# Audio-WestlakeU/FullSubNet

Measured on AMD Instinct MI355X. Metric: frames/sec (16 kHz, 512-FFT, hop 256), whole job, higher is better.
Workload: dtype f32

## Files before the change

fullsubnet_amd/csrc/fb_chain_kernels.hip:

```cpp
#include "fsn_common.h"

namespace {

constexpr int CHMAX = 512;
constexpr int CFS = CHMAX / 4;
constexpr int CREP = 16;

struct ChainArgs {
    const float* gx0;
    const float* whh0_p;
    const float* wih1_p;
    const float* whh1_p;
    const float* b1;
    float* hx0;
    float* hx1;
    float* gx1;
    float* hseq1;
    float* hseq0;
    float* gates0;
    float* cseq0;
    float* gates1;
    float* cseq1;
    unsigned* flags;
    unsigned* status;
    unsigned long long spin_ticks;
    int Tp, RT, Npad;
};

__device__ __forceinline__ bool chain_wait(const unsigned* flags, int nflags, unsigned epoch, const unsigned* one,
                                           unsigned one_epoch, unsigned* status, unsigned long long ticks) {
    const int lane = threadIdx.x & 63;
    const unsigned long long* f = reinterpret_cast<const unsigned long long*>(flags) + lane;
    unsigned long long t0 = 0;
    for (unsigned spins = 0;; ++spins) {
        unsigned long long v = ~0ull;
        unsigned w = ~0u;
        if (epoch > 0 && 2 * lane < nflags) v = __hip_atomic_load(f, __ATOMIC_RELAXED, __HIP_MEMORY_SCOPE_AGENT);
        if (one && lane == 0) w = __hip_atomic_load(one, __ATOMIC_RELAXED, __HIP_MEMORY_SCOPE_AGENT);
        if (__all((int)((unsigned)v >= epoch && (unsigned)(v >> 32) >= epoch && w >= one_epoch))) return true;
        if ((spins & 255u) == 255u && fsn_wait_give_up(status, spins, t0, ticks, 1u + epoch)) return false;
    }
}

typedef unsigned u32x4 __attribute__((ext_vector_type(4)));
__device__ __forceinline__ void chain_store16(const __amdgpu_buffer_rsrc_t& r, unsigned voff, unsigned soff, f32x4 v) {
    __builtin_amdgcn_raw_buffer_store_b128(__builtin_bit_cast(u32x4, v), r, voff, soff, 16);
}
template <int Q>
__device__ __forceinline__ float quad_bcast(float v) {
    return __builtin_bit_cast(float, __builtin_amdgcn_mov_dpp(__builtin_bit_cast(int, v), Q * 0x55, 0xf, 0xf, true));
}

template <int CH, int KS, bool SAVE = false, int CELL = 0>
__global__ __launch_bounds__(256, 1) void fb_chain_kernel(const ChainArgs a) {
    static_assert(!(SAVE && CELL != 0), "the training form is built for the LSTM cell");
    constexpr int CKC = CH / 16;
    constexpr int CNW = CH / 4;
    static_assert(CKC % 4 == 0 && CNW % 2 == 0 && CNW <= CFS, "hidden size: a multiple of 64, at most 512");
    constexpr int RTW = 4 / KS;
    constexpr int CW = CKC / KS;
    __shared__ f32x4 red[KS > 1 ? (KS - 1) * RTW * 64 : 1];

    const int stage = (int)blockIdx.x / CNW, j = (int)blockIdx.x % CNW;
    const int lane = threadIdx.x & 63, wave = __builtin_amdgcn_readfirstlane(threadIdx.x >> 6);
    const int rt = wave % RTW, kp = wave / RTW;
    const int lr = lane & 15, lq = lane >> 4, g = lr >> 2, ul = lr & 3;
    const int Tp = a.Tp, RT = a.RT;
    const bool active = rt < RT, owner = active && kp == 0;

    unsigned* fl0 = a.flags;
    unsigned* fl1 = a.flags + CREP * CFS;
    const int rep = j % CREP;

    const __amdgpu_buffer_rsrc_t r0 = __builtin_amdgcn_make_buffer_rsrc(a.hx0, 0, 0x7fffffff, 0x00020000);
    const __amdgpu_buffer_rsrc_t r1 = __builtin_amdgcn_make_buffer_rsrc(a.hx1, 0, 0x7fffffff, 0x00020000);
    const __amdgpu_buffer_rsrc_t rx = __builtin_amdgcn_make_buffer_rsrc(a.gx1, 0, 0x7fffffff, 0x00020000);
    const unsigned lane16 = (unsigned)lane * 16u;

    auto load_w = [&](const float* packed, f32x4 (&w)[CW]) {
        const float* wp = packed + ((size_t)(g * CKC + (j >> 2)) * CKC * 64 + lq * 16 + 4 * (j & 3) + ul) * 4;
#pragma unroll
        for (int q = 0; q < CW; ++q) w[q] = *reinterpret_cast<const f32x4*>(wp + (size_t)(kp * CW + q) * 256);
    };
    auto load_a = [&](f32x4 (&ar)[CW], const __amdgpu_buffer_rsrc_t& r, int ts) {
        const unsigned base = (unsigned)((((size_t)ts * RT + rt) * CKC + kp * CW) * 1024);
#pragma unroll
        for (int q = 0; q < CW; ++q)
            ar[q] = __builtin_bit_cast(f32x4, __builtin_amdgcn_raw_buffer_load_b128(r, lane16, base + q * 1024u, 16));
        __builtin_amdgcn_sched_barrier(0);
    };
    auto mac = [&](f32x4 acc, const f32x4 (&ar)[CW], const f32x4 (&w)[CW]) -> f32x4 {
#pragma unroll
        for (int q = 0; q < CW; ++q)
#pragma unroll
            for (int jj = 0; jj < 4; ++jj) acc = mfma16(ar[q][jj], w[q][jj], acc);
        return acc;
    };
    auto reduce = [&](f32x4 acc) -> f32x4 {
        if (KS > 1) {
            if (kp > 0) red[((kp - 1) * RTW + rt) * 64 + lane] = acc;
            __syncthreads();
            if (kp == 0) {
#pragma unroll
                for (int p = 1; p < KS; ++p) {
                    const f32x4 o = red[((p - 1) * RTW + rt) * 64 + lane];
                    acc = f32x4{acc[0] + o[0], acc[1] + o[1], acc[2] + o[2], acc[3] + o[3]};
                }
            }
        }
        return acc;
    };
    auto publish = [&](unsigned* flags, unsigned epoch) {
        asm volatile("s_waitcnt vmcnt(0)" ::: "memory");
        __syncthreads();
        if ((int)threadIdx.x < CREP)
            __hip_atomic_store(flags + (size_t)threadIdx.x * CFS + j, epoch, __ATOMIC_RELAXED, __HIP_MEMORY_SCOPE_AGENT);
    };
    auto quad_transpose = [&](const float (&v)[4]) -> f32x4 {
        f32x4 o;
#pragma unroll
        for (int u = 0; u < 4; ++u) {
            const float t0 = u == 0 ? quad_bcast<0>(v[0]) : u == 1 ? quad_bcast<1>(v[0]) : u == 2 ? quad_bcast<2>(v[0]) : quad_bcast<3>(v[0]);
            const float t1 = u == 0 ? quad_bcast<0>(v[1]) : u == 1 ? quad_bcast<1>(v[1]) : u == 2 ? quad_bcast<2>(v[1]) : quad_bcast<3>(v[1]);
            const float t2 = u == 0 ? quad_bcast<0>(v[2]) : u == 1 ? quad_bcast<1>(v[2]) : u == 2 ? quad_bcast<2>(v[2]) : quad_bcast<3>(v[2]);
            const float t3 = u == 0 ? quad_bcast<0>(v[3]) : u == 1 ? quad_bcast<1>(v[3]) : u == 2 ? quad_bcast<2>(v[3]) : quad_bcast<3>(v[3]);
            o[u] = ul == 0 ? t0 : ul == 1 ? t1 : ul == 2 ? t2 : t3;
        }
        return o;
    };
    const int hrow = 4 * lq + ul;
    auto cell = [&](f32x4 acc, float (&c)[4], float* gates_t, float* cseq_t) -> f32x4 {
        float act[4], hq[4];
        if constexpr (CELL == 1) {
#pragma unroll
            for (int i = 0; i < 4; ++i) {
                const float v = g < 2 ? sigmoid_f(acc[i]) : acc[i];
                const float z = __shfl(v, lane + 4, 64);
                const float nx = __shfl(v, lane + 8, 64);
                const float nh = __shfl(v, lane + 12, 64);
                const float n = tanhf(nx + v * nh);
                const float hn = n + z * (c[i] - n);
                c[i] = hn;
                hq[i] = hn;
            }
            return quad_transpose(hq);
        }
#pragma unroll
        for (int i = 0; i < 4; ++i) act[i] = g == 2 ? tanh_fast(acc[i]) : sigmoid_fast(acc[i]);
#pragma unroll
        for (int i = 0; i < 4; ++i) {
            const float fg = __shfl(act[i], lane + 4, 64);
            const float gg = __shfl(act[i], lane + 8, 64);
            const float og = __shfl(act[i], lane + 12, 64);
            const float cn = fg * c[i] + act[i] * gg;
            c[i] = cn;
            hq[i] = og * tanh_fast(cn);
        }
        if (SAVE) {
            const size_t row = (size_t)rt * 16 + hrow;
            *reinterpret_cast<f32x4*>(gates_t + row * (4 * CH) + g * CH + 4 * j) = quad_transpose(act);
            const f32x4 cv = quad_transpose(c);
            if (g == 0) *reinterpret_cast<f32x4*>(cseq_t + row * CH + 4 * j) = cv;
        }
        return quad_transpose(hq);
    };
    const unsigned hvoff = (unsigned)(((j & 3) * 16 + hrow) * 16);
    auto hsoff = [&](int t) { return (unsigned)((((size_t)t * RT + rt) * CKC + (j >> 2)) * 1024); };
    const unsigned gx1_wave = (unsigned)(((size_t)j * 4 + wave) * 1024);
    const unsigned gx1_step = (unsigned)CNW * 4096u;
    float c[4] = {0.f, 0.f, 0.f, 0.f};

    if (stage == 0) {
        f32x4 whh[CW], wih[CW], ar[CW];
        load_w(a.whh0_p, whh);
        load_w(a.wih1_p, wih);
        const float bias1 = a.b1[g * CH + 4 * j + ul];
        const float* gx0p = a.gx0 + ((size_t)(g * CKC + (j >> 2)) * 64 + lq * 16 + 4 * (j & 3) + ul) * 4 +
                            (size_t)rt * (4 * CKC) * 256;
        const size_t gx0_step = (size_t)RT * (4 * CKC) * 256;
        f32x4 gxn = f32x4{0.f, 0.f, 0.f, 0.f};
        if (owner) gxn = *reinterpret_cast<const f32x4*>(gx0p);
        for (int t = 0; t <= Tp; ++t) {
            f32x4 acc = gxn;
            if (owner && t + 1 < Tp) gxn = *reinterpret_cast<const f32x4*>(gx0p + (size_t)(t + 1) * gx0_step);
            if (t > 0) {
                if (wave == 0) (void)chain_wait(fl0 + rep * CFS, CNW, (unsigned)t, nullptr, 0, a.status, a.spin_ticks);
                __syncthreads();
                if (active) load_a(ar, r0, t - 1);
            }
            if (t < Tp) {
                if (active && t > 0) acc = mac(acc, ar, whh);
                acc = reduce(acc);
                if (owner) {
                    const f32x4 hv = cell(acc, c, SAVE ? a.gates0 + (size_t)t * a.Npad * 4 * CH : nullptr,
                                          SAVE ? a.cseq0 + (size_t)t * a.Npad * CH : nullptr);
                    if (g == 0) {
                        chain_store16(r0, hvoff, hsoff(t), hv);
                        if (SAVE) *reinterpret_cast<f32x4*>(a.hseq0 + ((size_t)t * a.Npad + rt * 16 + hrow) * CH + 4 * j) = hv;
                    }
                }
            }
            const bool proj = t > 0 && active;
            const float b = kp == 0 ? bias1 : 0.f;
            if (t < Tp) publish(fl0, (unsigned)t + 1);
            if (proj) {
                const f32x4 accx = mac(f32x4{b, b, b, b}, ar, wih);
                const unsigned so = (unsigned)(t - 1) * gx1_step + gx1_wave;
                asm volatile("buffer_store_dwordx4 %0, %1, %2, %3 offen sc1" ::"v"(accx), "v"(lane16), "s"(rx), "s"(so) : "memory");
            }
            if (t == Tp) publish(fl0, (unsigned)Tp + 2);
        }
        return;
    }

    f32x4 whh[CW], ar[CW];
    load_w(a.whh1_p, whh);
    for (int s = 0; s < Tp; ++s) {
        if (wave == 0)
            (void)chain_wait(fl1 + rep * CFS, CNW, (unsigned)s, fl0 + rep * CFS + j, (unsigned)s + 3, a.status, a.spin_ticks);
        __syncthreads();
        f32x4 acc = f32x4{0.f, 0.f, 0.f, 0.f};
        if (active) {
            acc = __builtin_bit_cast(f32x4, __builtin_amdgcn_raw_buffer_load_b128(rx, lane16, (unsigned)s * gx1_step + gx1_wave, 16));
            if (s > 0) {
                load_a(ar, r1, s - 1);
                acc = mac(acc, ar, whh);
            }
        }
        acc = reduce(acc);
        if (owner) {
            const f32x4 hv = cell(acc, c, SAVE ? a.gates1 + (size_t)s * a.Npad * 4 * CH : nullptr,
                                  SAVE ? a.cseq1 + (size_t)s * a.Npad * CH : nullptr);
            if (g == 0) {
                chain_store16(r1, hvoff, hsoff(s), hv);
                *reinterpret_cast<f32x4*>(a.hseq1 + ((size_t)s * a.Npad + rt * 16 + hrow) * CH + 4 * j) = hv;
            }
        }
        publish(fl1, (unsigned)s + 1);
    }
}

}

namespace {
template <int CH>
bool chain_grid_fits(int RT) {
    const unsigned grid = 2 * (CH / 4);
    const void *k, *ks;
    if (RT == 1) k = (const void*)fb_chain_kernel<CH, 4, false>, ks = (const void*)fb_chain_kernel<CH, 4, true>;
    else if (RT == 2) k = (const void*)fb_chain_kernel<CH, 2, false>, ks = (const void*)fb_chain_kernel<CH, 2, true>;
    else k = (const void*)fb_chain_kernel<CH, 1, false>, ks = (const void*)fb_chain_kernel<CH, 1, true>;
    const void* kg = RT == 1   ? (const void*)fb_chain_kernel<CH, 4, false, 1>
                     : RT == 2 ? (const void*)fb_chain_kernel<CH, 2, false, 1>
                               : (const void*)fb_chain_kernel<CH, 1, false, 1>;
    return fsn_grid_fits(k, 256, grid) && fsn_grid_fits(ks, 256, grid) && fsn_grid_fits(kg, 256, grid);
}
}
bool fsn_fb_chain_supported(int H, int Npad) {
    if ((H != 512 && H != 384) || Npad < 16 || Npad > 64 || Npad % 16 != 0) return false;
    if (!fsn_persistent_allowed()) return false;
    return H == 512 ? chain_grid_fits<512>(Npad / 16) : chain_grid_fits<384>(Npad / 16);
}
int fsn_fb_chain_max_steps() { return (int)(0x7fffffffu / ((unsigned)(CHMAX / 4) * 4096u)); }
size_t fsn_fb_chain_exchange_floats(int Tp, int Npad) {
    return (size_t)2 * Tp * Npad * CHMAX + (size_t)Tp * (CHMAX / 4) * 1024;
}
size_t fsn_fb_chain_flag_words() { return (size_t)2 * CREP * CFS + 16; }
size_t fsn_fb_chain_status_word() { return (size_t)2 * CREP * CFS; }

namespace {
template <int CH, bool SAVE, int CELL = 0>
void chain_launch(const ChainArgs& a, hipStream_t s) {
    const dim3 grid(2 * (CH / 4)), block(256);
    if (a.RT == 1) FSN_PERSIST_LAUNCH((fb_chain_kernel<CH, 4, SAVE, CELL>), grid, block, s, a);
    else if (a.RT == 2) FSN_PERSIST_LAUNCH((fb_chain_kernel<CH, 2, SAVE, CELL>), grid, block, s, a);
    else FSN_PERSIST_LAUNCH((fb_chain_kernel<CH, 1, SAVE, CELL>), grid, block, s, a);
}
}

int fsn_launch_fb_chain(const float* gx0, const float* whh0_p, const float* wih1_p, const float* whh1_p, const float* b1,
                        float* exchange, unsigned* flags, float* hseq1, int Tp, int Npad, int H, hipStream_t s,
                        float* hseq0, float* save0, float* save1, int cell) {
    if (!fsn_fb_chain_supported(H, Npad) || Tp < 1 || Tp > fsn_fb_chain_max_steps()) {
        fsn_set_error("fb_chain: built for H = 384 / 512, at most 64 rows and 4095 steps");
        return FSN_ERR_ARG;
    }
    const bool save = hseq0 || save0 || save1;
    if (cell != 0 && (cell != 1 || save)) {
        fsn_set_error("fb_chain: cell 0 (LSTM) or 1 (GRU as a four-gate cell, inference form only)");
        return FSN_ERR_ARG;
    }
    if (save && !(hseq0 && save0 && save1)) {
        fsn_set_error("fb_chain: the training form needs hseq0, save0 and save1");
        return FSN_ERR_ARG;
    }
    if (fsn_launch_zero_words(flags, fsn_fb_chain_flag_words(), s) != FSN_OK) return FSN_ERR_LAUNCH;
    ChainArgs a{};
    a.gx0 = gx0;
    a.whh0_p = whh0_p;
    a.wih1_p = wih1_p;
    a.whh1_p = whh1_p;
    a.b1 = b1;
    a.hx0 = exchange;
    a.hx1 = exchange + (size_t)Tp * Npad * H;
    a.gx1 = exchange + (size_t)2 * Tp * Npad * H;
    a.hseq1 = hseq1;
    a.hseq0 = hseq0;
    a.gates0 = save0;
    a.cseq0 = save0 ? save0 + (size_t)Tp * Npad * 4 * H : nullptr;
    a.gates1 = save1;
    a.cseq1 = save1 ? save1 + (size_t)Tp * Npad * 4 * H : nullptr;
    a.flags = flags;
    a.status = flags + fsn_fb_chain_status_word();
    a.spin_ticks = fsn_spin_ticks();
    a.Tp = Tp;
    a.RT = Npad / 16;
    a.Npad = Npad;
    if (H == 512) {
        if (cell) chain_launch<512, false, 1>(a, s);
        else if (save) chain_launch<512, true>(a, s);
        else chain_launch<512, false>(a, s);
    } else {
        if (cell) chain_launch<384, false, 1>(a, s);
        else if (save) chain_launch<384, true>(a, s);
        else chain_launch<384, false>(a, s);
    }
    return fsn_check_launch("fb_chain_kernel");
}
```

Before: 148,600.

## Pipeline row tiles through the two-layer chain with per-tile flags

For three or four row tiles, the chained two-layer recurrent kernel now uses a tile-rotating variant. Each wave owns one tile's cell update and publishes flags for that tile alone, so the next tile's wait and loads overlap the current tile's compute. The K split is reduced through shared memory with double buffering, and the layer-1 input projection is computed inside the layer-0 loop. The cell code is hoisted into a shared device function, and the flag array grows to hold per-tile flags. This adds more fine-grained synchronization and more complex slot bookkeeping.

```diff
diff --git a/fullsubnet_amd/csrc/fb_chain_kernels.hip b/fullsubnet_amd/csrc/fb_chain_kernels.hip
--- a/fullsubnet_amd/csrc/fb_chain_kernels.hip
+++ b/fullsubnet_amd/csrc/fb_chain_kernels.hip
@@ -5,6 +5,7 @@
 constexpr int CHMAX = 512;
 constexpr int CFS = CHMAX / 4;
 constexpr int CREP = 16;
+constexpr int CTILES = 4;
 
 struct ChainArgs {
     const float* gx0;
@@ -51,6 +52,57 @@
     return __builtin_bit_cast(float, __builtin_amdgcn_mov_dpp(__builtin_bit_cast(int, v), Q * 0x55, 0xf, 0xf, true));
 }
 
+__device__ __forceinline__ f32x4 chain_quad_transpose(const float (&v)[4], int ul) {
+    f32x4 o;
+#pragma unroll
+    for (int u = 0; u < 4; ++u) {
+        const float t0 = u == 0 ? quad_bcast<0>(v[0]) : u == 1 ? quad_bcast<1>(v[0]) : u == 2 ? quad_bcast<2>(v[0]) : quad_bcast<3>(v[0]);
+        const float t1 = u == 0 ? quad_bcast<0>(v[1]) : u == 1 ? quad_bcast<1>(v[1]) : u == 2 ? quad_bcast<2>(v[1]) : quad_bcast<3>(v[1]);
+        const float t2 = u == 0 ? quad_bcast<0>(v[2]) : u == 1 ? quad_bcast<1>(v[2]) : u == 2 ? quad_bcast<2>(v[2]) : quad_bcast<3>(v[2]);
+        const float t3 = u == 0 ? quad_bcast<0>(v[3]) : u == 1 ? quad_bcast<1>(v[3]) : u == 2 ? quad_bcast<2>(v[3]) : quad_bcast<3>(v[3]);
+        o[u] = ul == 0 ? t0 : ul == 1 ? t1 : ul == 2 ? t2 : t3;
+    }
+    return o;
+}
+
+template <int CH, bool SAVE, int CELL>
+__device__ __forceinline__ f32x4 chain_cell(f32x4 acc, float (&c)[4], float* gates_t, float* cseq_t, int rt, int j, int lane) {
+    const int lr = lane & 15, lq = lane >> 4, g = lr >> 2, ul = lr & 3;
+    float act[4], hq[4];
+    if constexpr (CELL == 1) {
+#pragma unroll
+        for (int i = 0; i < 4; ++i) {
+            const float v = g < 2 ? sigmoid_f(acc[i]) : acc[i];
+            const float z = __shfl(v, lane + 4, 64);
+            const float nx = __shfl(v, lane + 8, 64);
+            const float nh = __shfl(v, lane + 12, 64);
+            const float n = tanhf(nx + v * nh);
+            const float hn = n + z * (c[i] - n);
+            c[i] = hn;
+            hq[i] = hn;
+        }
+        return chain_quad_transpose(hq, ul);
+    }
+#pragma unroll
+    for (int i = 0; i < 4; ++i) act[i] = g == 2 ? tanh_fast(acc[i]) : sigmoid_fast(acc[i]);
+#pragma unroll
+    for (int i = 0; i < 4; ++i) {
+        const float fg = __shfl(act[i], lane + 4, 64);
+        const float gg = __shfl(act[i], lane + 8, 64);
+        const float og = __shfl(act[i], lane + 12, 64);
+        const float cn = fg * c[i] + act[i] * gg;
+        c[i] = cn;
+        hq[i] = og * tanh_fast(cn);
+    }
+    if (SAVE) {
+        const size_t row = (size_t)rt * 16 + 4 * lq + ul;
+        *reinterpret_cast<f32x4*>(gates_t + row * (4 * CH) + g * CH + 4 * j) = chain_quad_transpose(act, ul);
+        const f32x4 cv = chain_quad_transpose(c, ul);
+        if (g == 0) *reinterpret_cast<f32x4*>(cseq_t + row * CH + 4 * j) = cv;
+    }
+    return chain_quad_transpose(hq, ul);
+}
+
 template <int CH, int KS, bool SAVE = false, int CELL = 0>
 __global__ __launch_bounds__(256, 1) void fb_chain_kernel(const ChainArgs a) {
     static_assert(!(SAVE && CELL != 0), "the training form is built for the LSTM cell");
@@ -116,53 +168,9 @@
         if ((int)threadIdx.x < CREP)
             __hip_atomic_store(flags + (size_t)threadIdx.x * CFS + j, epoch, __ATOMIC_RELAXED, __HIP_MEMORY_SCOPE_AGENT);
     };
-    auto quad_transpose = [&](const float (&v)[4]) -> f32x4 {
-        f32x4 o;
-#pragma unroll
-        for (int u = 0; u < 4; ++u) {
-            const float t0 = u == 0 ? quad_bcast<0>(v[0]) : u == 1 ? quad_bcast<1>(v[0]) : u == 2 ? quad_bcast<2>(v[0]) : quad_bcast<3>(v[0]);
-            const float t1 = u == 0 ? quad_bcast<0>(v[1]) : u == 1 ? quad_bcast<1>(v[1]) : u == 2 ? quad_bcast<2>(v[1]) : quad_bcast<3>(v[1]);
-            const float t2 = u == 0 ? quad_bcast<0>(v[2]) : u == 1 ? quad_bcast<1>(v[2]) : u == 2 ? quad_bcast<2>(v[2]) : quad_bcast<3>(v[2]);
-            const float t3 = u == 0 ? quad_bcast<0>(v[3]) : u == 1 ? quad_bcast<1>(v[3]) : u == 2 ? quad_bcast<2>(v[3]) : quad_bcast<3>(v[3]);
-            o[u] = ul == 0 ? t0 : ul == 1 ? t1 : ul == 2 ? t2 : t3;
-        }
-        return o;
-    };
     const int hrow = 4 * lq + ul;
     auto cell = [&](f32x4 acc, float (&c)[4], float* gates_t, float* cseq_t) -> f32x4 {
-        float act[4], hq[4];
-        if constexpr (CELL == 1) {
-#pragma unroll
-            for (int i = 0; i < 4; ++i) {
-                const float v = g < 2 ? sigmoid_f(acc[i]) : acc[i];
-                const float z = __shfl(v, lane + 4, 64);
-                const float nx = __shfl(v, lane + 8, 64);
-                const float nh = __shfl(v, lane + 12, 64);
-                const float n = tanhf(nx + v * nh);
-                const float hn = n + z * (c[i] - n);
-                c[i] = hn;
-                hq[i] = hn;
-            }
-            return quad_transpose(hq);
-        }
-#pragma unroll
-        for (int i = 0; i < 4; ++i) act[i] = g == 2 ? tanh_fast(acc[i]) : sigmoid_fast(acc[i]);
-#pragma unroll
-        for (int i = 0; i < 4; ++i) {
-            const float fg = __shfl(act[i], lane + 4, 64);
-            const float gg = __shfl(act[i], lane + 8, 64);
-            const float og = __shfl(act[i], lane + 12, 64);
-            const float cn = fg * c[i] + act[i] * gg;
-            c[i] = cn;
-            hq[i] = og * tanh_fast(cn);
-        }
-        if (SAVE) {
-            const size_t row = (size_t)rt * 16 + hrow;
-            *reinterpret_cast<f32x4*>(gates_t + row * (4 * CH) + g * CH + 4 * j) = quad_transpose(act);
-            const f32x4 cv = quad_transpose(c);
-            if (g == 0) *reinterpret_cast<f32x4*>(cseq_t + row * CH + 4 * j) = cv;
-        }
-        return quad_transpose(hq);
+        return chain_cell<CH, SAVE, CELL>(acc, c, gates_t, cseq_t, rt, j, lane);
     };
     const unsigned hvoff = (unsigned)(((j & 3) * 16 + hrow) * 16);
     auto hsoff = [&](int t) { return (unsigned)((((size_t)t * RT + rt) * CKC + (j >> 2)) * 1024); };
@@ -240,19 +248,195 @@
     }
 }
 
+__device__ __forceinline__ bool chain_wait_part(const unsigned* f, int n, unsigned epoch, const unsigned* one,
+                                                unsigned one_epoch, unsigned* status, unsigned long long ticks) {
+    const int lane = threadIdx.x & 63;
+    unsigned long long t0 = 0;
+    bool ok = false;
+    for (unsigned spins = 0;; ++spins) {
+        unsigned v = ~0u, w = ~0u;
+        if (epoch > 0 && lane < n) v = __hip_atomic_load(f + lane, __ATOMIC_RELAXED, __HIP_MEMORY_SCOPE_AGENT);
+        if (one && lane == 63) w = __hip_atomic_load(one, __ATOMIC_RELAXED, __HIP_MEMORY_SCOPE_AGENT);
+        if (__all((int)(v >= epoch && w >= one_epoch))) { ok = true; break; }
+        if ((spins & 255u) == 255u && fsn_wait_give_up(status, spins, t0, ticks, 1u + epoch)) break;
+    }
+    __builtin_amdgcn_fence(__ATOMIC_ACQUIRE, "wavefront");
+    asm volatile("" ::: "memory");
+    return ok;
+}
+
+template <int CH, bool SAVE = false, int CELL = 0>
+__global__ __launch_bounds__(256, 1) void fb_chain_tiles_kernel(const ChainArgs a) {
+    static_assert(!(SAVE && CELL != 0), "the training form is built for the LSTM cell");
+    constexpr int CKC = CH / 16;
+    constexpr int CNW = CH / 4;
+    constexpr int CW = CKC / 4;
+    constexpr int NP = CNW / 4;
+    static_assert(CKC % 4 == 0 && CNW <= CFS && NP <= 63, "hidden size: a multiple of 64, at most 512");
+    __shared__ f32x4 red[2][4][64];
+    __shared__ f32x4 redp[2][4][64];
+
+    const int stage = (int)blockIdx.x / CNW, j = (int)blockIdx.x % CNW;
+    const int lane = threadIdx.x & 63, kp = __builtin_amdgcn_readfirstlane(threadIdx.x >> 6);
+    const int lr = lane & 15, lq = lane >> 4, g = lr >> 2, ul = lr & 3;
+    const int Tp = a.Tp, NT = a.RT;
+    const int rep = j % CREP;
+    auto tile_flags = [&](int st, int tile) { return a.flags + (size_t)((st * CTILES + tile) * CREP) * CFS; };
+
+    const __amdgpu_buffer_rsrc_t r0 = __builtin_amdgcn_make_buffer_rsrc(a.hx0, 0, 0x7fffffff, 0x00020000);
+    const __amdgpu_buffer_rsrc_t r1 = __builtin_amdgcn_make_buffer_rsrc(a.hx1, 0, 0x7fffffff, 0x00020000);
+    const __amdgpu_buffer_rsrc_t rx = __builtin_amdgcn_make_buffer_rsrc(a.gx1, 0, 0x7fffffff, 0x00020000);
+    const unsigned lane16 = (unsigned)lane * 16u;
+
+    auto load_w = [&](const float* packed, f32x4 (&w)[CW]) {
+        const float* wp = packed + ((size_t)(g * CKC + (j >> 2)) * CKC * 64 + lq * 16 + 4 * (j & 3) + ul) * 4;
+#pragma unroll
+        for (int q = 0; q < CW; ++q) w[q] = *reinterpret_cast<const f32x4*>(wp + (size_t)(kp * CW + q) * 256);
+    };
+    auto load_a = [&](f32x4 (&ar)[CW], const __amdgpu_buffer_rsrc_t& r, int ts, int tile) {
+        const unsigned base = (unsigned)((((size_t)ts * NT + tile) * CKC + kp * CW) * 1024);
+#pragma unroll
+        for (int q = 0; q < CW; ++q)
+            ar[q] = __builtin_bit_cast(f32x4, __builtin_amdgcn_raw_buffer_load_b128(r, lane16, base + q * 1024u, 16));
+    };
+    auto mac = [&](f32x4 acc, const f32x4 (&ar)[CW], const f32x4 (&w)[CW]) -> f32x4 {
+#pragma unroll
+        for (int q = 0; q < CW; ++q)
+#pragma unroll
+            for (int jj = 0; jj < 4; ++jj) acc = mfma16(ar[q][jj], w[q][jj], acc);
+        return acc;
+    };
+    auto sum4 = [&](const f32x4 (&p)[4][64]) -> f32x4 {
+        f32x4 acc = p[0][lane];
+#pragma unroll
+        for (int q = 1; q < 4; ++q) {
+            const f32x4 o = p[q][lane];
+            acc = f32x4{acc[0] + o[0], acc[1] + o[1], acc[2] + o[2], acc[3] + o[3]};
+        }
+        return acc;
+    };
+    auto publish = [&](int st, int tile, unsigned epoch) {
+        if (lane < CREP)
+            __hip_atomic_store(tile_flags(st, tile) + (size_t)lane * CFS + j, epoch, __ATOMIC_RELAXED, __HIP_MEMORY_SCOPE_AGENT);
+    };
+    const int hrow = 4 * lq + ul;
+    const unsigned hvoff = (unsigned)(((j & 3) * 16 + hrow) * 16);
+    auto hsoff = [&](int t, int tile) { return (unsigned)((((size_t)t * NT + tile) * CKC + (j >> 2)) * 1024); };
+    auto gx1off = [&](int t, int tile) { return (unsigned)t * ((unsigned)CNW * 4096u) + (unsigned)((j * 4 + tile) * 1024); };
+    float c[4] = {0.f, 0.f, 0.f, 0.f};
+    f32x4 ar[CW], an[CW] = {};
+    f32x4 gc, gn = f32x4{0.f, 0.f, 0.f, 0.f};
+
+    if (stage == 0) {
+        f32x4 whh[CW], wih[CW];
+        load_w(a.whh0_p, whh);
+        load_w(a.wih1_p, wih);
+        const float bias1 = kp == 0 ? a.b1[g * CH + 4 * j + ul] : 0.f;
+        const float* gx0p = a.gx0 + ((size_t)(g * CKC + (j >> 2)) * 64 + lq * 16 + 4 * (j & 3) + ul) * 4;
+        auto gx0_at = [&](int t, int tile) {
+            return *reinterpret_cast<const f32x4*>(gx0p + ((size_t)t * NT + tile) * (4 * CKC) * 256);
+        };
+        if (kp == 0) gn = gx0_at(0, 0);
+        const int nslots = (Tp + 1) * NT;
+        int t = 0, r = 0, tq = 0, rq = 0;
+        for (int k = 0; k < nslots; ++k) {
+            int t1 = t, r1 = r + 1;
+            if (r1 == NT) r1 = 0, t1 = t + 1;
+            asm volatile("s_waitcnt vmcnt(0)" ::: "memory");
+            if (k > 0 && tq < Tp && kp == rq) publish(0, rq, (unsigned)tq + 1);
+#pragma unroll
+            for (int q = 0; q < CW; ++q) ar[q] = an[q];
+            gc = gn;
+            if (t1 <= Tp) {
+                if (t1 > 0) {
+                    (void)chain_wait_part(tile_flags(0, r1) + rep * CFS + kp * NP, NP, (unsigned)t1, nullptr, 0, a.status, a.spin_ticks);
+                    load_a(an, r0, t1 - 1, r1);
+                }
+                if (kp == 0 && t1 < Tp) gn = gx0_at(t1, r1);
+            }
+            const int par = k & 1;
+            if (t < Tp) {
+                f32x4 acc = kp == 0 ? gc : f32x4{0.f, 0.f, 0.f, 0.f};
+                if (t > 0) acc = mac(acc, ar, whh);
+                red[par][kp][lane] = acc;
+            }
+            __syncthreads();
+            if (k > 0 && tq > 0 && kp == rq) chain_store16(rx, lane16, gx1off(tq - 1, rq), sum4(redp[par ^ 1]));
+            if (t < Tp && kp == r) {
+                const f32x4 hv = chain_cell<CH, SAVE, CELL>(sum4(red[par]), c, SAVE ? a.gates0 + (size_t)t * a.Npad * 4 * CH : nullptr,
+                                                            SAVE ? a.cseq0 + (size_t)t * a.Npad * CH : nullptr, r, j, lane);
+                if (g == 0) {
+                    chain_store16(r0, hvoff, hsoff(t, r), hv);
+                    if (SAVE) *reinterpret_cast<f32x4*>(a.hseq0 + ((size_t)t * a.Npad + r * 16 + hrow) * CH + 4 * j) = hv;
+                }
+            }
+            if (t > 0) redp[par][kp][lane] = mac(f32x4{bias1, bias1, bias1, bias1}, ar, wih);
+            tq = t, rq = r, t = t1, r = r1;
+        }
+        __syncthreads();
+        if (kp == rq) chain_store16(rx, lane16, gx1off(tq - 1, rq), sum4(redp[(nslots - 1) & 1]));
+        asm volatile("s_waitcnt vmcnt(0)" ::: "memory");
+        __syncthreads();
+        if (kp < NT) publish(0, kp, (unsigned)Tp + 2);
+        return;
+    }
+
+    f32x4 whh[CW];
+    load_w(a.whh1_p, whh);
+    auto request = [&](int s, int tile) {
+        (void)chain_wait_part(tile_flags(1, tile) + rep * CFS + kp * NP, NP, (unsigned)s, tile_flags(0, tile) + rep * CFS + j,
+                              (unsigned)s + 3, a.status, a.spin_ticks);
+        if (kp == 0) gn = __builtin_bit_cast(f32x4, __builtin_amdgcn_raw_buffer_load_b128(rx, lane16, gx1off(s, tile), 16));
+        if (s > 0) load_a(an, r1, s - 1, tile);
+    };
+    request(0, 0);
+    const int nslots = Tp * NT;
+    int s = 0, r = 0, sq = 0, rq = 0;
+    for (int k = 0; k < nslots; ++k) {
+        int s1 = s, rn = r + 1;
+        if (rn == NT) rn = 0, s1 = s + 1;
+        asm volatile("s_waitcnt vmcnt(0)" ::: "memory");
+        if (k > 0 && kp == rq) publish(1, rq, (unsigned)sq + 1);
+#pragma unroll
+        for (int q = 0; q < CW; ++q) ar[q] = an[q];
+        gc = gn;
+        if (k + 1 < nslots) request(s1, rn);
+        const int par = k & 1;
+        f32x4 acc = kp == 0 ? gc : f32x4{0.f, 0.f, 0.f, 0.f};
+        if (s > 0) acc = mac(acc, ar, whh);
+        red[par][kp][lane] = acc;
+        __syncthreads();
+        if (kp == r) {
+            const f32x4 hv = chain_cell<CH, SAVE, CELL>(sum4(red[par]), c, SAVE ? a.gates1 + (size_t)s * a.Npad * 4 * CH : nullptr,
+                                                        SAVE ? a.cseq1 + (size_t)s * a.Npad * CH : nullptr, r, j, lane);
+            if (g == 0) {
+                chain_store16(r1, hvoff, hsoff(s, r), hv);
+                *reinterpret_cast<f32x4*>(a.hseq1 + ((size_t)s * a.Npad + r * 16 + hrow) * CH + 4 * j) = hv;
+            }
+        }
+        sq = s, rq = r, s = s1, r = rn;
+    }
+    asm volatile("s_waitcnt vmcnt(0)" ::: "memory");
+    if (kp == rq) publish(1, rq, (unsigned)sq + 1);
+}
+
 }
 
 namespace {
 template <int CH>
 bool chain_grid_fits(int RT) {
     const unsigned grid = 2 * (CH / 4);
-    const void *k, *ks;
-    if (RT == 1) k = (const void*)fb_chain_kernel<CH, 4, false>, ks = (const void*)fb_chain_kernel<CH, 4, true>;
-    else if (RT == 2) k = (const void*)fb_chain_kernel<CH, 2, false>, ks = (const void*)fb_chain_kernel<CH, 2, true>;
-    else k = (const void*)fb_chain_kernel<CH, 1, false>, ks = (const void*)fb_chain_kernel<CH, 1, true>;
-    const void* kg = RT == 1   ? (const void*)fb_chain_kernel<CH, 4, false, 1>
-                     : RT == 2 ? (const void*)fb_chain_kernel<CH, 2, false, 1>
-                               : (const void*)fb_chain_kernel<CH, 1, false, 1>;
+    const void *k, *ks, *kg;
+    if (RT == 1) {
+        k = (const void*)fb_chain_kernel<CH, 4, false>, ks = (const void*)fb_chain_kernel<CH, 4, true>;
+        kg = (const void*)fb_chain_kernel<CH, 4, false, 1>;
+    } else if (RT == 2) {
+        k = (const void*)fb_chain_kernel<CH, 2, false>, ks = (const void*)fb_chain_kernel<CH, 2, true>;
+        kg = (const void*)fb_chain_kernel<CH, 2, false, 1>;
+    } else {
+        k = (const void*)fb_chain_tiles_kernel<CH, false>, ks = (const void*)fb_chain_tiles_kernel<CH, true>;
+        kg = (const void*)fb_chain_tiles_kernel<CH, false, 1>;
+    }
     return fsn_grid_fits(k, 256, grid) && fsn_grid_fits(ks, 256, grid) && fsn_grid_fits(kg, 256, grid);
 }
 }
@@ -265,8 +449,8 @@
 size_t fsn_fb_chain_exchange_floats(int Tp, int Npad) {
     return (size_t)2 * Tp * Npad * CHMAX + (size_t)Tp * (CHMAX / 4) * 1024;
 }
-size_t fsn_fb_chain_flag_words() { return (size_t)2 * CREP * CFS + 16; }
-size_t fsn_fb_chain_status_word() { return (size_t)2 * CREP * CFS; }
+size_t fsn_fb_chain_flag_words() { return (size_t)2 * CTILES * CREP * CFS + 16; }
+size_t fsn_fb_chain_status_word() { return (size_t)2 * CTILES * CREP * CFS; }
 
 namespace {
 template <int CH, bool SAVE, int CELL = 0>
@@ -274,7 +458,7 @@
     const dim3 grid(2 * (CH / 4)), block(256);
     if (a.RT == 1) FSN_PERSIST_LAUNCH((fb_chain_kernel<CH, 4, SAVE, CELL>), grid, block, s, a);
     else if (a.RT == 2) FSN_PERSIST_LAUNCH((fb_chain_kernel<CH, 2, SAVE, CELL>), grid, block, s, a);
-    else FSN_PERSIST_LAUNCH((fb_chain_kernel<CH, 1, SAVE, CELL>), grid, block, s, a);
+    else FSN_PERSIST_LAUNCH((fb_chain_tiles_kernel<CH, SAVE, CELL>), grid, block, s, a);
 }
 }
 
```

Result: slower. 146,800 (-1.2%).
